# orottier/web-audio-api-rs

Hardware: AMD Instinct MI355X
Metric: render quanta/sec (48kHz, 128-frame) (higher is better)
Workload: dtype f64

## Files before the change

### web-audio-api-rs_amd/csrc/waa_biquad_stream.hip

```cpp
#include <hip/hip_runtime.h>

#include <cstdlib>

#include "waa_internal.hpp"
#include "waa_stream_common.hpp"

namespace waa {

namespace {
struct M2 {
  double a, b, c, d;
};
__device__ __forceinline__ M2 mm(const M2& x, const M2& y) {
  M2 r;
  r.a = __builtin_fma(x.a, y.a, x.b * y.c);
  r.b = __builtin_fma(x.a, y.b, x.b * y.d);
  r.c = __builtin_fma(x.c, y.a, x.d * y.c);
  r.d = __builtin_fma(x.c, y.b, x.d * y.d);
  return r;
}

}

__device__ unsigned long long g_stream_trace[8192 * 4];

template <int DBG, int VARY, int NBUF = 2, bool DUP = false>
__global__ __launch_bounds__(64, 2) void biquad_stream_kernel_t(const BiquadStreamDesc d) {
  extern __shared__ __attribute__((aligned(16))) float lds[];
  const uint32_t wid = blockIdx.x;
  const uint32_t inst = wid / (uint32_t)d.nch;
  const int ch = (int)(wid % (uint32_t)d.nch);
  const int lane = threadIdx.x;
  if (inst >= d.n_inst) return;

  __builtin_amdgcn_s_setreg(1 | (6 << 6) | (1 << 11), 0);
  unsigned long long trace_t0 = 0;
  if constexpr (DBG == 7) trace_t0 = wall_clock64();

  const double* cp = d.coefs + (uint64_t)inst * d.coef_stride;
  double b0 = cp[0], b1 = cp[1], b2 = cp[2], a1 = cp[3], a2 = cp[4];
  M2 A1;
  {
    M2 m = {-a1, -a2, 1., 0.};
#pragma unroll
    for (int s = 0; s < 5; s++) m = mm(m, m);
    A1 = m;
  }
  const M2 A2 = mm(A1, A1), A4 = mm(A2, A2), A8 = mm(A4, A4), A16 = mm(A8, A8);
  M2 Aj = {1., 0., 0., 1.};
  if constexpr (VARY == 0) {
    const int j = lane & 15;
    if (j & 1) Aj = mm(Aj, A1);
    if (j & 2) Aj = mm(Aj, A2);
    if (j & 4) Aj = mm(Aj, A4);
    if (j & 8) Aj = mm(Aj, A8);
  }
  const int row = lane >> 4;

  double* st = d.state + (uint64_t)inst * STATE_STRIDE + ch * 4;
  double cx1 = st[0], cx2 = st[1], cy1 = st[2], cy2 = st[3];

  float g[2] = {1.f, 1.f};
  bool g_mute[2] = {false, false}, g_pass[2] = {true, true};
#pragma unroll
  for (int k = 0; k < 2; k++)
    if (k < d.n_gain) {
      g[k] = d.gain[k].base[inst];
      g_mute[k] = fabsf(g[k]) <= 1e-6f;
      g_pass[k] = fabsf(1.f - g[k]) <= 1e-6f;
    }

  const bool is_src = d.in.kind == IN_SOURCE;
  SrcInst si{};
  SrcSchedule sc{};
  const float* sig_base = nullptr;
  if (is_src) {
    si = d.in.src[inst];
    sc = si.sc;
  } else {
    sig_base = d.in.sig.base + (uint64_t)inst * d.in.sig.inst_stride + (uint64_t)ch * d.in.sig.ch_stride;
  }
  float* out_base = d.out.base + (uint64_t)inst * d.out.inst_stride + (uint64_t)ch * d.out.ch_stride;

  auto lds_sync = []() __attribute__((always_inline)) { __builtin_amdgcn_wave_barrier(); };

  auto fetch_fast = [&](uint32_t tile, float (&dst)[TILE_K]) __attribute__((always_inline)) {
    const float* p = is_src ? si.base + (uint64_t)ch * si.ch_stride +
                                  (tile < si.fast_prefix ? si.linear_start + (int64_t)tile * TILE
                                                         : load_global(&sc.qrec[(uint64_t)tile * QUANTA_PER_TILE].start))
                            : sig_base + (uint64_t)tile * TILE;
#pragma unroll
    for (int j = 0; j < NV4; j++) {
      const f4v t = DBG == 5 ? load_global_f4(p + j * 256 + lane * 4)
                             : __builtin_nontemporal_load((const WAA_GLOBAL_AS f4v*)(p + j * 256 + lane * 4));
      dst[j * 4 + 0] = t.x;
      dst[j * 4 + 1] = t.y;
      dst[j * 4 + 2] = t.z;
      dst[j * 4 + 3] = t.w;
    }
  };
  auto tile_is_fast = [&](uint32_t tile) __attribute__((always_inline)) -> bool {
    return !is_src || tile < si.fast_prefix || (si.aligned && load_global(sc.tile_fast + tile));
  };

  auto stage = [&](const float (&cur)[TILE_K]) __attribute__((always_inline)) {
#pragma unroll
    for (int j = 0; j < NV4; j++) {
      const int r = j * 8 + (lane >> 3), c = (lane & 7) * 4;
      *reinterpret_cast<float4*>(lds + r * LDS_ROW + c) =
          make_float4(cur[j * 4 + 0], cur[j * 4 + 1], cur[j * 4 + 2], cur[j * 4 + 3]);
    }
  };
  float* lds_out = lds + 64 * LDS_ROW;
  auto flush = [&](uint32_t tile) __attribute__((always_inline)) {
    lds_sync();
    float* op = out_base + (uint64_t)tile * TILE;
#pragma unroll
    for (int j = 0; j < NV4; j++) {
      const int r = j * 8 + (lane >> 3), c = (lane & 7) * 4;
      float4 t = *reinterpret_cast<const float4*>(lds_out + r * LDS_ROW + c);
#pragma unroll
      for (int k = 0; k < 2; k++)
        if (k < d.n_gain) {
          if (g_mute[k]) {
            t = make_float4(0.f, 0.f, 0.f, 0.f);
          } else if (!g_pass[k]) {
            t.x *= g[k];
            t.y *= g[k];
            t.z *= g[k];
            t.w *= g[k];
          }
        }
      if constexpr (DBG == 2) {
        asm volatile("" ::"v"(t.x), "v"(t.y), "v"(t.z), "v"(t.w));
      } else if constexpr (DBG == 5) {
        *reinterpret_cast<float4*>(op + j * 256 + lane * 4) = t;
      } else {
        __builtin_nontemporal_store(f4v{t.x, t.y, t.z, t.w}, (WAA_GLOBAL_AS f4v*)(op + j * 256 + lane * 4));
        if constexpr (DUP)
          __builtin_nontemporal_store(f4v{t.x, t.y, t.z, t.w}, (WAA_GLOBAL_AS f4v*)(op + d.out.ch_stride + j * 256 + lane * 4));
      }
    }
    lds_sync();
  };
  auto process_arate = [&](uint32_t tile) __attribute__((always_inline)) {
    lds_sync();
    const float* xrow = lds + lane * LDS_ROW;
    float* yrow = lds_out + lane * LDS_ROW;
    const double* ct = cp + (uint64_t)tile * (TILE_K * 5 * 64) + lane;
    auto load_chunk = [&](double (&c)[20], int chunk) __attribute__((always_inline)) {
      if (DBG >= 3 && tile != d.tile0) return;
#pragma unroll
      for (int j = 0; j < 20; j++) c[j] = load_global(ct + (chunk * 20 + j) * 64);
    };
    const float xl1 = xrow[TILE_K - 1], xl2 = xrow[TILE_K - 2];
    const float xm1 = __shfl_up(xl1, 1, 64), xm2 = __shfl_up(xl2, 1, 64);
    const double xs1 = lane == 0 ? cx1 : (double)xm1, xs2 = lane == 0 ? cx2 : (double)xm2;
    double x1 = xs1, x2 = xs2, z1 = 0., z2 = 0.;
    M2 P = {1., 0., 0., 1.};
    double ca[20], cb[20], cc[NBUF == 3 ? 20 : 1];
    if constexpr (VARY == 3) {
      const double* hp = d.hp + (uint64_t)(DBG == 4 ? d.tile0 : tile) * (HP_WORDS * 64) + lane;
      load_chunk(ca, 0);
      load_chunk(cb, 1);
      double za = load_global(hp + 64 * 64) * xs1, zb = load_global(hp + 65 * 64) * xs1;
      double zc = load_global(hp + 66 * 64) * xs2, zd = load_global(hp + 67 * 64) * xs2;
#pragma unroll 2
      for (int chunk = 0; chunk < TILE_K / 4; chunk++) {
        const float4 xv = *reinterpret_cast<const float4*>(xrow + chunk * 4);
        const double* hc = hp + chunk * 8 * 64;
        const double h0 = load_global(hc), h1 = load_global(hc + 64), h2 = load_global(hc + 128), h3 = load_global(hc + 192),
                     h4 = load_global(hc + 256), h5 = load_global(hc + 320), h6 = load_global(hc + 384), h7 = load_global(hc + 448);
        za = __builtin_fma(h0, (double)xv.x, za);
        zb = __builtin_fma(h1, (double)xv.x, zb);
        zc = __builtin_fma(h2, (double)xv.y, zc);
        zd = __builtin_fma(h3, (double)xv.y, zd);
        za = __builtin_fma(h4, (double)xv.z, za);
        zb = __builtin_fma(h5, (double)xv.z, zb);
        zc = __builtin_fma(h6, (double)xv.w, zc);
        zd = __builtin_fma(h7, (double)xv.w, zd);
      }
      z1 = za + zc;
      z2 = zb + zd;
      P.a = load_global(hp + 68 * 64);
      P.b = load_global(hp + 69 * 64);
// ... 82 lines not shown
            p2 = p1;
            p1 = xd2;
            double y = (wi - c[j * 5 + 3] * y1) - c[j * 5 + 4] * y2;
            if (flush_bad && !__builtin_isnormal(y)) y = 0.;
            y2 = y1;
            y1 = y;
            yo[j] = (float)y;
            badacc = __builtin_fmaf(yo[j], 0.f, badacc);
          }
          *reinterpret_cast<float4*>(yrow + chunk * 4) = make_float4(yo[0], yo[1], yo[2], yo[3]);
        };
        if constexpr (NBUF == 3) {
#pragma unroll 1
          for (int chunk = 0; chunk < 6; chunk += 3) {
            load_chunk(cc, chunk + 2);
            step_b(ca, chunk);
            load_chunk(ca, chunk + 3);
            step_b(cb, chunk + 1);
            load_chunk(cb, chunk + 4);
            step_b(cc, chunk + 2);
          }
          step_b(ca, 6);
          step_b(cb, 7);
        } else {
#pragma unroll 1
          for (int chunk = 0; chunk < TILE_K / 4; chunk += 2) {
            step_b(ca, chunk);
            if (chunk + 2 < TILE_K / 4) load_chunk(ca, chunk + 2);
            step_b(cb, chunk + 1);
            if (chunk + 3 < TILE_K / 4) load_chunk(cb, chunk + 3);
          }
        }
      };
      sweep(false);
      if (__any(badacc != badacc)) {
        y1 = __builtin_isfinite(s1) ? s1 : 0.;
        y2 = __builtin_isfinite(s2) ? s2 : 0.;
        load_chunk(ca, 0);
        load_chunk(cb, 1);
        sweep(true);
      }
      cx1 = (double)__int_as_float(__builtin_amdgcn_readlane(__float_as_int(xl1), 63));
      cx2 = (double)__int_as_float(__builtin_amdgcn_readlane(__float_as_int(xl2), 63));
      cy1 = read_lane(y1, 63);
      cy2 = read_lane(y2, 63);
    }
    lds_sync();
  };
  auto process = [&](uint32_t tile) __attribute__((always_inline)) {
    lds_sync();
    float x[TILE_K];
#pragma unroll
    for (int j = 0; j < NV4; j++) {
      const float4 t = *reinterpret_cast<const float4*>(lds + lane * LDS_ROW + j * 4);
      x[j * 4 + 0] = t.x;
      x[j * 4 + 1] = t.y;
      x[j * 4 + 2] = t.z;
      x[j * 4 + 3] = t.w;
    }
    if constexpr (DBG == 1) {
      lds_sync();
#pragma unroll
      for (int j = 0; j < NV4; j++)
        *reinterpret_cast<float4*>(lds_out + lane * LDS_ROW + j * 4) =
            make_float4(x[j * 4 + 0], x[j * 4 + 1], x[j * 4 + 2], x[j * 4 + 3]);
      lds_sync();
      return;
    }
    M2 Al = A1;
    if constexpr (VARY == 1) {
      uint32_t q = tile * QUANTA_PER_TILE + (lane >> 2);
      if (q >= d.n_quanta) q = d.n_quanta - 1;
      const double* cq = cp + (uint64_t)q * 5;
      b0 = cq[0];
      b1 = cq[1];
      b2 = cq[2];
      a1 = cq[3];
      a2 = cq[4];
      M2 m = {-a1, -a2, 1., 0.};
#pragma unroll
      for (int s = 0; s < 5; s++) m = mm(m, m);
      Al = m;
    }
    const float xm1 = __shfl_up(x[TILE_K - 1], 1, 64), xm2 = __shfl_up(x[TILE_K - 2], 1, 64);
    double x1 = lane == 0 ? cx1 : (double)xm1;
    double x2 = lane == 0 ? cx2 : (double)xm2;
    double w[TILE_K];
    double z1 = 0., z2 = 0.;
#pragma unroll
    for (int i = 0; i < TILE_K; i++) {
      const double xd = (double)x[i];
      w[i] = (b0 * xd + b1 * x1) + b2 * x2;
      x2 = x1;
      x1 = xd;
      const double t = __builtin_fma(-a2, z2, w[i]);
      const double y = __builtin_fma(-a1, z1, t);
      z2 = z1;
      z1 = y;
    }
    double s1, s2;
    if constexpr (VARY == 0) {
      double r1 = z1, r2 = z2;
      {
        double q1 = row_shr<1>(r1), q2 = row_shr<1>(r2);
        r1 = __builtin_fma(A1.a, q1, __builtin_fma(A1.b, q2, r1));
        r2 = __builtin_fma(A1.c, q1, __builtin_fma(A1.d, q2, r2));
        q1 = row_shr<2>(r1);
        q2 = row_shr<2>(r2);
        r1 = __builtin_fma(A2.a, q1, __builtin_fma(A2.b, q2, r1));
        r2 = __builtin_fma(A2.c, q1, __builtin_fma(A2.d, q2, r2));
        q1 = row_shr<4>(r1);
        q2 = row_shr<4>(r2);
        r1 = __builtin_fma(A4.a, q1, __builtin_fma(A4.b, q2, r1));
        r2 = __builtin_fma(A4.c, q1, __builtin_fma(A4.d, q2, r2));
        q1 = row_shr<8>(r1);
        q2 = row_shr<8>(r2);
        r1 = __builtin_fma(A8.a, q1, __builtin_fma(A8.b, q2, r1));
        r2 = __builtin_fma(A8.c, q1, __builtin_fma(A8.d, q2, r2));
      }
      const double e01 = read_lane(r1, 15), e02 = read_lane(r2, 15);
      const double e11 = read_lane(r1, 31), e12 = read_lane(r2, 31);
      const double e21 = read_lane(r1, 47), e22 = read_lane(r2, 47);
      const double t01 = cy1, t02 = cy2;
      const double t11 = __builtin_fma(A16.a, t01, __builtin_fma(A16.b, t02, e01));
      const double t12 = __builtin_fma(A16.c, t01, __builtin_fma(A16.d, t02, e02));
      const double t21 = __builtin_fma(A16.a, t11, __builtin_fma(A16.b, t12, e11));
      const double t22 = __builtin_fma(A16.c, t11, __builtin_fma(A16.d, t12, e12));
      const double t31 = __builtin_fma(A16.a, t21, __builtin_fma(A16.b, t22, e21));
      const double t32 = __builtin_fma(A16.c, t21, __builtin_fma(A16.d, t22, e22));
      const double T1 = row == 0 ? t01 : row == 1 ? t11 : row == 2 ? t21 : t31;
      const double T2 = row == 0 ? t02 : row == 1 ? t12 : row == 2 ? t22 : t32;
      const double ex1 = row_shr<1>(r1), ex2 = row_shr<1>(r2);
      s1 = __builtin_fma(Aj.a, T1, __builtin_fma(Aj.b, T2, ex1));
      s2 = __builtin_fma(Aj.c, T1, __builtin_fma(Aj.d, T2, ex2));
    } else {
      M2 P = Al;
      double r1 = z1, r2 = z2;
      auto step = [&](auto shr) __attribute__((always_inline)) {
        M2 Q;
        Q.a = shr(P.a, 1.);
        Q.b = shr(P.b, 0.);
        Q.c = shr(P.c, 0.);
        Q.d = shr(P.d, 1.);
        const double q1 = shr(r1, 0.), q2 = shr(r2, 0.);
        r1 = __builtin_fma(P.a, q1, __builtin_fma(P.b, q2, r1));
        r2 = __builtin_fma(P.c, q1, __builtin_fma(P.d, q2, r2));
        P = mm(P, Q);
      };
      step([](double v, double idv) __attribute__((always_inline)) { return row_shr_keep<1>(v, idv); });
      step([](double v, double idv) __attribute__((always_inline)) { return row_shr_keep<2>(v, idv); });
      step([](double v, double idv) __attribute__((always_inline)) { return row_shr_keep<4>(v, idv); });
      step([](double v, double idv) __attribute__((always_inline)) { return row_shr_keep<8>(v, idv); });
      double t1[4], t2[4];
      t1[0] = cy1;
      t2[0] = cy2;
#pragma unroll
      for (int k = 0; k < 3; k++) {
        const int e = 16 * k + 15;
        const double pa = read_lane(P.a, e), pb = read_lane(P.b, e), pc = read_lane(P.c, e), pd = read_lane(P.d, e);
        const double e1 = read_lane(r1, e), e2 = read_lane(r2, e);
        t1[k + 1] = __builtin_fma(pa, t1[k], __builtin_fma(pb, t2[k], e1));
        t2[k + 1] = __builtin_fma(pc, t1[k], __builtin_fma(pd, t2[k], e2));
      }
      const double T1 = row == 0 ? t1[0] : row == 1 ? t1[1] : row == 2 ? t1[2] : t1[3];
      const double T2 = row == 0 ? t2[0] : row == 1 ? t2[1] : row == 2 ? t2[2] : t2[3];
      const double xa = row_shr_keep<1>(P.a, 1.), xb = row_shr_keep<1>(P.b, 0.), xc = row_shr_keep<1>(P.c, 0.),
                   xd = row_shr_keep<1>(P.d, 1.);
      const double x1r = row_shr_keep<1>(r1, 0.), x2r = row_shr_keep<1>(r2, 0.);
      s1 = __builtin_fma(xa, T1, __builtin_fma(xb, T2, x1r));
      s2 = __builtin_fma(xc, T1, __builtin_fma(xd, T2, x2r));
    }
    double y1 = s1, y2 = s2;
    float badacc = 0.f;
    float yo[TILE_K];
#pragma unroll
    for (int i = 0; i < TILE_K; i++) {
      const double y = (w[i] - a1 * y1) - a2 * y2;
      y2 = y1;
      y1 = y;
      yo[i] = (float)y;
      badacc = __builtin_fmaf(yo[i], 0.f, badacc);
    }
    if (__any(badacc != badacc)) {
      y1 = s1;
      y2 = s2;
      if (!__builtin_isfinite(y1)) y1 = 0.;
      if (!__builtin_isfinite(y2)) y2 = 0.;
#pragma unroll
      for (int i = 0; i < TILE_K; i++) {
        double y = (w[i] - a1 * y1) - a2 * y2;
        if (!__builtin_isnormal(y)) y = 0.;
        y2 = y1;
        y1 = y;
        yo[i] = (float)y;
      }
    }
    cx1 = (double)__int_as_float(__builtin_amdgcn_readlane(__float_as_int(x[TILE_K - 1]), 63));
    cx2 = (double)__int_as_float(__builtin_amdgcn_readlane(__float_as_int(x[TILE_K - 2]), 63));
    cy1 = read_lane(y1, 63);
    cy2 = read_lane(y2, 63);
    lds_sync();
#pragma unroll
    for (int j = 0; j < NV4; j++)
      *reinterpret_cast<float4*>(lds_out + lane * LDS_ROW + j * 4) =
          make_float4(yo[j * 4 + 0], yo[j * 4 + 1], yo[j * 4 + 2], yo[j * 4 + 3]);
    lds_sync();
  };

  bool pending = false;
  uint32_t pending_tile = 0;
  uint32_t tile = d.tile0;
  while (tile < d.tile1) {
    if (!tile_is_fast(tile)) {
      float tmp[TILE_K];
      load_channel_generic(d.in, si, sc, ch, tile, lane, d.n_quanta, tmp);
      float cur[TILE_K];
#pragma unroll
      for (int i = 0; i < TILE_K; i++) cur[i] = tmp[i];
      stage(cur);
      if (pending) flush(pending_tile);
      if constexpr (VARY >= 2) process_arate(tile); else process(tile);
      pending = true;
      pending_tile = tile;
      tile++;
      continue;
    }
    uint32_t end = tile + 1;
    if (is_src && end < si.fast_prefix) end = si.fast_prefix < d.tile1 ? si.fast_prefix : d.tile1;
    while (end < d.tile1 && tile_is_fast(end)) end++;
    if constexpr (VARY == 0 && NBUF == 4) {
      float na[TILE_K], nb[TILE_K];
      fetch_fast(tile, na);
      fetch_fast(tile + 1 < end ? tile + 1 : tile, nb);
      for (; tile + 1 < end; tile += 2) {
        stage(na);
        fetch_fast(tile + 2 < end ? tile + 2 : tile, na);
        if (pending) flush(pending_tile);
        process(tile);
        pending = true;
        pending_tile = tile;
        stage(nb);
        fetch_fast(tile + 3 < end ? tile + 3 : tile + 1, nb);
        flush(pending_tile);
        process(tile + 1);
        pending_tile = tile + 1;
      }
      if (tile < end) {
        stage(na);
        if (pending) flush(pending_tile);
        process(tile);
        pending = true;
        pending_tile = tile;
        tile++;
      }
      continue;
    }
    float nx[TILE_K];
    fetch_fast(tile, nx);
    for (; tile < end; tile++) {
      stage(nx);
      fetch_fast(tile + 1 < end ? tile + 1 : tile, nx);
      if (pending) flush(pending_tile);
      if constexpr (VARY >= 2) process_arate(tile); else process(tile);
      pending = true;
      pending_tile = tile;
    }
  }
  if (pending) flush(pending_tile);
  if (lane == 0) {
    st[0] = cx1;
    st[1] = cx2;
    st[2] = cy1;
    st[3] = cy2;
  }
  if constexpr (DBG == 7) {
    if (lane == 0 && wid < 8192) {
      g_stream_trace[wid * 4 + 0] = trace_t0;
      g_stream_trace[wid * 4 + 1] = wall_clock64();
      g_stream_trace[wid * 4 + 2] = __builtin_amdgcn_s_getreg(4 | (0 << 6) | (31 << 11));
      g_stream_trace[wid * 4 + 3] = __builtin_amdgcn_s_getreg(20 | (0 << 6) | (31 << 11));
    }
  }
}

__global__ __launch_bounds__(64, 4) void biquad_stream_digest_kernel(const BiquadStreamDesc d) {
  extern __shared__ __attribute__((aligned(16))) float lds[];
  double* htab = reinterpret_cast<double*>(lds + 64 * LDS_ROW);
  const uint32_t wid = blockIdx.x;
  const uint32_t inst = wid / (uint32_t)d.nch;
  const int ch = (int)(wid % (uint32_t)d.nch);
  const int lane = threadIdx.x;
  if (inst >= d.n_inst) return;
  __builtin_amdgcn_s_setreg(1 | (6 << 6) | (1 << 11), 0);

  auto uni = [](double v) __attribute__((always_inline)) {
    return __hiloint2double(__builtin_amdgcn_readfirstlane(__double2hiint(v)), __builtin_amdgcn_readfirstlane(__double2loint(v)));
  };
  auto uni_m = [&](const M2& m) __attribute__((always_inline)) { return M2{uni(m.a), uni(m.b), uni(m.c), uni(m.d)}; };
  const double* cp = d.coefs + (uint64_t)inst * d.coef_stride;
  const double b0 = uni(cp[0]), b1 = uni(cp[1]), b2 = uni(cp[2]), a1 = uni(cp[3]), a2 = uni(cp[4]);
  M2 A1;
  {
    M2 m = {-a1, -a2, 1., 0.};
#pragma unroll
    for (int s = 0; s < 5; s++) m = mm(m, m);
    A1 = uni_m(m);
  }
  const M2 A2 = uni_m(mm(A1, A1)), A4 = uni_m(mm(A2, A2)), A8 = uni_m(mm(A4, A4)), A16 = uni_m(mm(A8, A8));
  M2 Aj = {1., 0., 0., 1.};
  {
    const int j = lane & 15;
    if (j & 1) Aj = mm(Aj, A1);
    if (j & 2) Aj = mm(Aj, A2);
    if (j & 4) Aj = mm(Aj, A4);
    if (j & 8) Aj = mm(Aj, A8);
  }
  const int row = lane >> 4;
  {
    double g1 = 1., g2 = 0.;
    double p1 = 0., p2 = 0.;
    double q1 = 0., q2 = 0.;
    double h1 = 0., h2 = 0.;
    for (int n = 0; n < TILE_K; n++) {
      if (lane == TILE_K - 1 - n) {
        h1 = __builtin_fma(b0, g1, __builtin_fma(b1, p1, b2 * q1));
        h2 = __builtin_fma(b0, g2, __builtin_fma(b1, p2, b2 * q2));
      }
      if (n == TILE_K - 1) {
        if (lane == 32) {
          h1 = __builtin_fma(b1, g1, b2 * p1);
          h2 = __builtin_fma(b1, g2, b2 * p2);
        }
        if (lane == 33) {
          h1 = b2 * g1;
          h2 = b2 * g2;
        }
      }
      const double n1 = __builtin_fma(-a1, g1, -(a2 * g2)), n2 = g1;
      q1 = p1;
      q2 = p2;
      p1 = g1;
      p2 = g2;
      g1 = n1;
      g2 = n2;
    }
    if (lane < 34) {
      htab[lane * 2] = h1;
      htab[lane * 2 + 1] = h2;
    }
  }
  double* st = d.state + (uint64_t)inst * STATE_STRIDE + ch * 4;
  double cx1 = st[0], cx2 = st[1], cy1 = st[2], cy2 = st[3];
  float g[2] = {1.f, 1.f};
  bool g_mute[2] = {false, false}, g_pass[2] = {true, true};
#pragma unroll
  for (int k = 0; k < 2; k++)
    if (k < d.n_gain) {
      g[k] = d.gain[k].base[inst];
      g_mute[k] = fabsf(g[k]) <= 1e-6f;
      g_pass[k] = fabsf(1.f - g[k]) <= 1e-6f;
    }
  const bool is_src = d.in.kind == IN_SOURCE;
  SrcInst si{};
  SrcSchedule sc{};
  const float* sig_base = nullptr;
// ... 159 lines not shown
      }
      if (__any(badacc != badacc)) {
        y1 = sy1;
        y2 = sy2;
        p1 = sp1;
        p2 = sp2;
#pragma unroll
        for (int j = 0; j < 4; j++) {
          const double xd = (double)xf[j];
          const double wi = (b0 * xd + b1 * p1) + b2 * p2;
          p2 = p1;
          p1 = xd;
          double y = (wi - a1 * y1) - a2 * y2;
          if (!__builtin_isnormal(y)) y = 0.;
          y2 = y1;
          y1 = y;
          yo[j] = (float)y;
        }
      }
      *reinterpret_cast<float4*>(xrow + c * 4) = make_float4(yo[0], yo[1], yo[2], yo[3]);
    }
    cx1 = (double)__int_as_float(__builtin_amdgcn_readlane(__float_as_int(xl1), 63));
    cx2 = (double)__int_as_float(__builtin_amdgcn_readlane(__float_as_int(xl2), 63));
    cy1 = read_lane(y1, 63);
    cy2 = read_lane(y2, 63);
  };
  bool have = false;
  uint32_t done = 0;
  uint32_t tile = d.tile0;
  while (tile < d.tile1) {
    if (!tile_is_fast(tile)) {
      float tmp[TILE_K];
      load_channel_generic(d.in, si, sc, ch, tile, lane, d.n_quanta, tmp);
      float cur[TILE_K];
#pragma unroll
      for (int i = 0; i < TILE_K; i++) cur[i] = tmp[i];
      swap_in(cur, have, done);
      process();
      have = true;
      done = tile;
      tile++;
      continue;
    }
    uint32_t end = tile + 1;
    if (is_src && end < si.fast_prefix) end = si.fast_prefix < d.tile1 ? si.fast_prefix : d.tile1;
    while (end < d.tile1 && tile_is_fast(end)) end++;
    float nx[TILE_K];
    fetch_fast(tile, nx);
    for (; tile < end; tile++) {
      swap_in(nx, have, done);
      fetch_fast(tile + 1 < end ? tile + 1 : tile, nx);
      process();
      have = true;
      done = tile;
    }
  }
  if (have) flush_last(done);
  if (lane == 0) {
    st[0] = cx1;
    st[1] = cx2;
    st[2] = cy1;
    st[3] = cy2;
  }
}

void launch_biquad_stream(const BiquadStreamDesc& d, void* stream) {
  const dim3 grid(d.n_inst * (uint32_t)d.nch), block(64);
  const size_t lds = 2 * 64 * LDS_ROW * sizeof(float);
  const char* dbg = measure_switch("WAA_STREAM_DEBUG");
  if (d.dup_out && d.vary == 0) {
    hipLaunchKernelGGL((biquad_stream_kernel_t<0, 0, 4, true>), grid, block, lds, (hipStream_t)stream, d);
    return;
  }
  if (d.vary == 3 && dbg && dbg[0] == '3')
    hipLaunchKernelGGL((biquad_stream_kernel_t<3, 3>), grid, block, lds, (hipStream_t)stream, d);
  else if (d.vary == 3 && dbg && dbg[0] == '4')
    hipLaunchKernelGGL((biquad_stream_kernel_t<4, 3>), grid, block, lds, (hipStream_t)stream, d);
  else if (d.vary == 3 && measure_switch("WAA_ARATE_BUFS3"))
    hipLaunchKernelGGL((biquad_stream_kernel_t<0, 3, 3>), grid, block, lds, (hipStream_t)stream, d);
  else if (d.vary == 3)
    hipLaunchKernelGGL((biquad_stream_kernel_t<0, 3>), grid, block, lds, (hipStream_t)stream, d);
  else if (d.vary == 2)
    hipLaunchKernelGGL((biquad_stream_kernel_t<0, 2>), grid, block, lds, (hipStream_t)stream, d);
  else if (d.vary)
    hipLaunchKernelGGL((biquad_stream_kernel_t<0, 1>), grid, block, lds, (hipStream_t)stream, d);
  else if (dbg && dbg[0] == '1')
    hipLaunchKernelGGL((biquad_stream_kernel_t<1, 0>), grid, block, lds, (hipStream_t)stream, d);
  else if (dbg && dbg[0] == '2')
    hipLaunchKernelGGL((biquad_stream_kernel_t<2, 0>), grid, block, lds, (hipStream_t)stream, d);
  else if (dbg && dbg[0] == '5')
    hipLaunchKernelGGL((biquad_stream_kernel_t<5, 0>), grid, block, lds, (hipStream_t)stream, d);
  else if (dbg && dbg[0] == '7')
    hipLaunchKernelGGL((biquad_stream_kernel_t<7, 0>), grid, block, lds, (hipStream_t)stream, d);
  else if (measure_switch("WAA_STREAM_PREFETCH1"))
    hipLaunchKernelGGL((biquad_stream_kernel_t<0, 0, 2>), grid, block, lds, (hipStream_t)stream, d);
  else if (measure_switch("WAA_BIQUAD_DIGEST"))
    hipLaunchKernelGGL(biquad_stream_digest_kernel, grid, block, 64 * LDS_ROW * sizeof(float) + 34 * 2 * sizeof(double),
                       (hipStream_t)stream, d);
  else
    hipLaunchKernelGGL((biquad_stream_kernel_t<0, 0, 4>), grid, block, lds, (hipStream_t)stream, d);
}

}

extern "C" int waa_debug_stream_trace(unsigned long long* dst, unsigned n_words) {
  return (int)hipMemcpyFromSymbol(dst, HIP_SYMBOL(waa::g_stream_trace), (size_t)n_words * 8);
}
```

### web-audio-api-rs_amd/csrc/waa_internal.hpp

```cpp
#pragma once
#include <cstdint>
#include <cstdlib>

#include "waa_conv_noise.hpp"

namespace waa {

inline const char* measure_switch(const char* name) {
#ifdef WAA_MEASURE
  return getenv(name);
#else
  (void)name;
  return nullptr;
#endif
}

void raise_lds_limit(const void* kernel);

constexpr int RQ = 128;
constexpr int TILE_K = 32;
constexpr int TILE = 64 * TILE_K;
constexpr int QUANTA_PER_TILE = TILE / RQ;
constexpr int MAX_OPS = 12;
constexpr int MAX_INPUTS = 4;
// ... 37 lines not shown
  uint64_t frames;
  uint32_t sched;
  uint32_t aligned;
  SrcSchedule sc;
  int64_t linear_start;
  uint32_t fast_prefix;
  uint32_t linear_all;
};

enum : int32_t { IN_SILENT = 0, IN_SIGNAL = 1, IN_SOURCE = 2, IN_CONSTANT = 3, IN_DELAYED = 4 };
struct InputRef {
  int32_t kind;
  int32_t nch;
  SignalRef sig;
  const SrcInst* src;
  const SrcSchedule* sched;
  ParamRef offset;
  const int64_t* active;
  double sample_rate;
  int32_t num_quanta;
  int32_t feedback;
  uint64_t valid;
  ParamRef gain;
  int32_t has_gain;
  uint32_t fast_tiles;
  float delay_lo, delay_hi;
};

enum : int32_t {
  OP_GAIN = 1,
  OP_BIQUAD = 2,
  OP_WAVESHAPER = 3,
  OP_STEREO_PAN = 4,
  OP_PANNER = 5,
  OP_MIX = 6,
  OP_IIR = 7,
  OP_PARAM_ADD = 8
};
struct OpDesc {
  int32_t kind;
  int32_t nch_in;
  int32_t nch_out;
  int32_t i1;
  int32_t i2;
  int32_t i0;
  ParamRef p0;
  ParamRef p1;
  ParamRef p2;
  ParamRef p3;
  ParamRef p4;
  const void* ptr0;
  void* ptr1;
  const void* ptr2;
  uint64_t u0;
};

struct ChainDesc {
  int32_t n_inputs;
  int32_t in_nch;
  int32_t in_interp;
  int32_t n_ops;
  InputRef in[MAX_INPUTS];
  OpDesc ops[MAX_OPS];
  SignalRef out;
  uint32_t n_inst;
  uint32_t n_tiles;
  uint32_t n_quanta;
  uint32_t xcd_remap;
  uint32_t tile0, tile1;
  int32_t lds_curve_op;
  int32_t tile_major;
  uint32_t persist_block;
  uint32_t pad;
};

struct BiquadStreamDesc {
  InputRef in;
  const double* coefs;
  uint64_t coef_stride;
  int32_t vary;
  int32_t pad0;
  double* state;
  const double* hp;
  ParamRef gain[2];
  int32_t n_gain;
  int32_t nch;
  SignalRef out;
  uint32_t n_inst;
  uint32_t n_tiles;
  uint32_t n_quanta;
  uint32_t dup_out;
  uint32_t tile0, tile1;
};
void launch_biquad_stream(const BiquadStreamDesc& d, void* stream);
constexpr int BIQUAD_SCAN_PW = 88;
struct BiquadScanCtl {
  uint32_t* counter;
  uint32_t counter_base[8];
  double* payload;
  const double* pw;
  uint32_t* error;
};
void launch_biquad_scan_powers(const double* coefs, uint64_t coef_stride, double* pw, uint32_t n_inst, void* stream);
void launch_biquad_scan(const BiquadStreamDesc& d, const BiquadScanCtl& ctl, uint32_t* issued, void* stream);

constexpr int BIQUAD_HT_WORDS = 2 * TILE + 8;
struct BiquadLanesDesc {
  InputRef in;
  const double* coefs;
  double* ht;
  double* z;
  double* sin;
  double* state;
  ParamRef gain[2];
  int32_t n_gain, nch;
  SignalRef out;
  uint32_t n_inst, n_tiles, n_quanta, tile0, tile1;
  uint32_t fast_tiles;
  uint32_t lt0, lt1;
  uint32_t debug, pad;
};
void launch_biquad_tile_digest(const BiquadLanesDesc& d, void* stream);
void launch_biquad_lanes(const BiquadLanesDesc& d, void* stream);

struct IirStreamDesc {
  InputRef in;
  const double* coef;
  const double* pow;
  double* state;
  int32_t ns;
  int32_t nch;
  SignalRef out;
  uint32_t n_inst;
  uint32_t n_tiles;
  uint32_t n_quanta;
  uint32_t exact;
  uint32_t tile0, tile1;
};
int iir_padded_states(int n_states);
void launch_iir_stream(const IirStreamDesc& d, void* stream);

struct CompRow {
  float thr, lo, hi, half_knee;
  float knee_partial, ratio, makeup, pad;
  float a_tau, a_one, r_tau, r_one;
};
struct CompDesc {
  SignalRef in;
  uint64_t in_valid;
  SignalRef out;
  float* xl;
  const CompRow* rows;
  uint32_t row_inst_stride, row_q_stride;
  uint32_t n_inst, n_quanta;
  uint64_t frames;
  uint32_t delay_frames;
  int32_t nch;
};
void launch_compressor_level(const CompDesc& d, void* stream);
void launch_compressor_detector(const CompDesc& d, void* stream);
void launch_compressor_apply(const CompDesc& d, void* stream);

enum : int32_t { RT_CHANNEL = 0, RT_DOWN2 = 1, RT_DOWN4 = 2, RT_DOWN6 = 3 };
struct RouteTerm {
  const float* base;
  uint64_t inst_stride, ch_stride;
  int32_t mode;
  int32_t ch;
};
struct RouteDesc {
  SignalRef out;
  const RouteTerm* terms;
  const uint32_t* row_off;
  uint32_t n_inst, rows;
  uint64_t frames;
};
void launch_route(const RouteDesc& d, void* stream);
// ... 514 lines not shown
```

### web-audio-api-rs_amd/csrc/waa_plan.cpp

```cpp
#include <array>
#include <set>

#include <memory>

#include "waa_host.hpp"
#include "waa_plan_parts.hpp"

namespace waa {
namespace host {

int prepare_source_input(waa_batch* b, uint32_t id, InputRef* in);
int validate_plan(waa_batch* b);

int device_timeline_param(waa_batch* b, const ParamStore& p, ParamRef* ref) {
  if (p.dev_ready) {
    *ref = p.dev_ref;
    return 0;
  }
  std::vector<TlHeader> hdr(b->n_inst);
  std::vector<TlEvent> events;
  std::vector<float> curves;
  for (uint32_t i = 0; i < b->n_inst; i++) {
    TlHeader& h = hdr[i];
    std::memset(&h, 0, sizeof h);
// ... 675 lines not shown
      in.kind = IN_SIGNAL;
      in.nch = cur_nch;
      in.sig = seg_out;
      inputs.assign(1, in);
      in_nch = cur_nch;
      i = j;
      if (i == ops.size() && seg_out.base == out.base) return 0;
      continue;
    }
    if (o.kind == OP_BIQUAD && o.i0 == 2 && !dup && b->steps[(size_t)o.i1].coef.rows == 1 && !measure_switch("WAA_ARATE_STREAM") &&
        (inputs[0].kind == IN_SIGNAL || inputs[0].kind == IN_SOURCE) &&
        (uint64_t)b->n_inst * seg_out.inst_stride < (1ull << 32)) {
      Step& cstep = b->steps[(size_t)o.i1];
      Step& dstep = b->steps[(size_t)o.i1 + 1];
      cstep.coef.lane_major = 0;
      const size_t n_streams = (size_t)b->n_inst * cur_nch;
      double *ht = nullptr, *z = nullptr, *sin = nullptr;
      int e;
      if ((e = dev_alloc(b, &ht, (size_t)b->n_tiles * BIQUAD_HT_WORDS)) || (e = dev_alloc(b, &z, (size_t)b->n_tiles * n_streams * 2)) ||
          (e = dev_alloc(b, &sin, (size_t)b->n_tiles * n_streams * 2)))
        return e;
      BiquadLanesDesc L;
      std::memset(&L, 0, sizeof L);
      L.in = inputs[0];
      L.coefs = cstep.coef.coefs;
      L.ht = ht;
      L.z = z;
      L.sin = sin;
      L.state = reinterpret_cast<double*>(o.ptr1);
      L.n_gain = (int)(j - i - 1);
      for (size_t k = i + 1; k < j; k++) L.gain[k - i - 1] = ops[k].p0;
      L.nch = cur_nch;
      L.out = seg_out;
      L.n_inst = b->n_inst;
      L.n_tiles = b->n_tiles;
      L.n_quanta = b->n_quanta;
      L.tile0 = 0;
      L.tile1 = b->n_tiles;
      L.fast_tiles = inputs[0].kind == IN_SOURCE ? inputs[0].fast_tiles
                                                 : (inputs[0].valid ? (uint32_t)std::min<uint64_t>(inputs[0].valid / TILE, b->n_tiles) : b->n_tiles);
      dstep.kind = 18;
      dstep.lanes = L;
      dstep.profile_slot = slot_for(b, "biquad_tile_digest_kernel");
      Step ls;
      ls.kind = 19;
      ls.lanes = L;
      ls.profile_slot = slot_for(b, "biquad_lanes_kernel");
      b->steps.push_back(ls);
      plan_note(b, "biquad_lanes(a-rate, shared table: one lane per stream, tiles in parallel) in=%s:%dch gains=%d out=%s",
                input_kind_name(inputs[0].kind), cur_nch, L.n_gain, seg_out.base == out.base ? "final" : "temp");
      InputRef in{};
      in.kind = IN_SIGNAL;
      in.nch = cur_nch;
      in.sig = seg_out;
      inputs.assign(1, in);
      in_nch = cur_nch;
      i = j;
      if (i == ops.size() && seg_out.base == out.base) return 0;
      continue;
    }
    Step st;
    st.kind = 1;
    BiquadStreamDesc& q = st.bq;
    std::memset(&q, 0, sizeof q);
    q.in = inputs[0];
    q.coefs = reinterpret_cast<const double*>(o.ptr0);
    q.coef_stride = o.u0;
    q.vary = o.i0;
    if (o.i0 == 2) {
      Step& cstep = b->steps[(size_t)o.i1];
      cstep.coef.lane_major = 1;
      if (cstep.coef.rows == 1 && !measure_switch("WAA_NO_ARATE_DIGEST")) {
        Step& hstep = b->steps[(size_t)o.i1 + 1];
        double* dhp = nullptr;
        int e = dev_alloc(b, &dhp, (size_t)b->n_tiles * HP_WORDS * 64);
        if (e) return e;
        hstep.hp.coefs = cstep.coef.coefs;
        hstep.hp.hp = dhp;
        hstep.hp.n_tiles = b->n_tiles;
        q.hp = dhp;
        q.vary = 3;
      }
    }
    q.state = reinterpret_cast<double*>(o.ptr1);
    q.n_gain = (int)(j - i - 1);
    for (size_t k = i + 1; k < j; k++) q.gain[k - i - 1] = ops[k].p0;
    q.nch = cur_nch;
    q.out = seg_out;
    q.dup_out = dup ? 1u : 0u;
    q.n_inst = b->n_inst;
    q.n_tiles = b->n_tiles;
    q.tile0 = 0;
    q.tile1 = b->n_tiles;
    q.n_quanta = b->n_quanta;
    st.profile_slot = slot_for(b, "biquad_stream_kernel");
    if (q.vary == 0 && !b->dry && measure_switch("WAA_BIQUAD_SCAN")) {
      const size_t n_streams = (size_t)b->n_inst * cur_nch;
      if (!b->scan_counter) {
        int e = dev_alloc(b, &b->scan_counter, 8 * 16 + 16);
        if (e) return e;
        b->state_bufs.push_back({b->scan_counter, (8 * 16 + 16) * sizeof(uint32_t)});
      }
      double *payload = nullptr, *pw = nullptr;
      int e;
      if ((e = dev_alloc(b, &payload, n_streams * b->n_tiles * 8)) || (e = dev_alloc(b, &pw, (size_t)b->n_inst * BIQUAD_SCAN_PW)))
        return e;
      b->ones_bufs.push_back({payload, n_streams * b->n_tiles * 8 * sizeof(double)});
      launch_biquad_scan_powers(q.coefs, q.coef_stride, pw, b->n_inst, b->stream);
      HIP_TRY(hipGetLastError());
      st.scan.counter = b->scan_counter;
      st.scan.error = b->scan_counter + 8 * 16;
      st.scan.payload = payload;
      st.scan.pw = pw;
      st.profile_slot = slot_for(b, "biquad_scan_kernel");
    }
    b->steps.push_back(st);
    if (dup) {
      plan_note(b, "biquad_stream in=%s:1ch gains=%d out=final (both channels: the speakers up-mix 1 -> 2 behind it)",
                input_kind_name(inputs[0].kind), q.n_gain);
      return 0;
    }
    plan_note(b, "biquad_stream%s in=%s:%dch gains=%d out=%s",
              q.vary == 3 ? "(a-rate, shared table)" : q.vary == 2 ? "(a-rate, per-instance table)" : q.vary ? "(k-rate)" : "",
              input_kind_name(inputs[0].kind),
              cur_nch, q.n_gain, seg_out.base == out.base ? "final" : "temp");
    InputRef in{};
    in.kind = IN_SIGNAL;
    in.nch = cur_nch;
    in.sig = seg_out;
    inputs.assign(1, in);
    in_nch = cur_nch;
    i = j;
    if (i == ops.size() && seg_out.base == out.base) return 0;
  }
  return push_chain_step(b, inputs, in_nch, in_interp, pending, out);
}

bool is_delay(const waa_batch* b, uint32_t id) { return b->nodes[id].desc.kind == WAA_NODE_DELAY; }
void vertex_targets(const waa_batch* b, uint32_t v, const std::vector<uint8_t>& cut, std::vector<uint32_t>& out) {
  const uint32_t id = v & ~VTX_READER;
  if (!(v & VTX_READER) && is_delay(b, id)) {
    if (!cut[id]) out.push_back(id | VTX_READER);
    return;
  }
  for (auto& e : b->edges) {
    if (e.from != id) continue;
    out.push_back(is_delay(b, e.to) && (e.to_input & 0x80000000u) ? (e.to | VTX_READER) : e.to);
  }
}

int materialise_automation(waa_batch* b) {
  const double sample_rate = (double)b->sr, dt = 1. / sample_rate;
  for (Node& n : b->nodes)
    for (size_t pk = 0; pk < n.params.size(); pk++) {
      ParamStore& p = n.params[pk];
      if (p.timelines.empty()) continue;
      bool shared = p.timelines_shared && p.timelines[0];
      for (uint32_t i = 1; i < b->n_inst && shared; i++) shared = p.cst[i] == p.cst[0] && p.timelines[i];
      {
        const uint32_t kind = n.desc.kind;
        const bool consumable = kind == WAA_NODE_GAIN || kind == WAA_NODE_BIQUAD || kind == WAA_NODE_DELAY ||
                                kind == WAA_NODE_STEREO_PANNER || kind == WAA_NODE_CONSTANT_SOURCE ||
                                kind == WAA_NODE_OSCILLATOR ||
                                (kind == WAA_NODE_PANNER && pk >= 6 && n.desc.i[0] != WAA_PANNING_HRTF);
        const bool want = measure_switch("WAA_DEVICE_AUTOMATION") ? true : !shared;
        bool arrivals = false;
// ... 1312 lines not shown
```

### web-audio-api-rs_amd/csrc/waa_plan_ops.cpp

```cpp
#include <array>
#include <set>

#include "waa_host.hpp"
#include "waa_plan_parts.hpp"

namespace waa {
namespace host {

int emit_node_ops(waa_batch* b, uint32_t id, int cur_nch, bool head, std::vector<OpDesc>& ops, int* out_nch) {
  Node& n = b->nodes[id];
  const uint32_t kind = n.desc.kind;
  if (kind == WAA_NODE_BUFFER_SOURCE || kind == WAA_NODE_CONSTANT_SOURCE) {
    *out_nch = n.out_nch;
    return 0;
  }
  if (!head && cur_nch != n.in_nch) {
    OpDesc m{};
    m.kind = OP_MIX;
    m.nch_in = cur_nch;
    m.nch_out = n.in_nch;
    m.i0 = n.interp;
    ops.push_back(m);
  }
  const int nch = n.in_nch;
  *out_nch = n.out_nch;
  switch (kind) {
    case WAA_NODE_GAIN: {
      OpDesc o{};
      o.kind = OP_GAIN;
      o.nch_in = o.nch_out = nch;
      int e = node_param(b, id, 0, &o.p0);
      if (e) return e;
      ops.push_back(o);
      break;
    }
    case WAA_NODE_BIQUAD: {
      OpDesc o{};
      o.kind = OP_BIQUAD;
      o.nch_in = o.nch_out = nch;
      bool varies = false, a_rate = false;
      for (size_t k = 0; k < n.params.size(); k++) {
        if (param_mode(n, k) == 2) a_rate = true;
        if (param_mode(n, k) == 1) varies = true;
      }
      if (a_rate) {
        Step cs;
        cs.kind = 5;
        BiquadCoefDesc& cdsc = cs.coef;
        std::memset(&cdsc, 0, sizeof cdsc);
        int e;
        if ((e = node_param(b, id, WAA_PARAM_BIQUAD_FREQUENCY, &cdsc.frequency)) ||
            (e = node_param(b, id, WAA_PARAM_BIQUAD_DETUNE, &cdsc.detune)) ||
            (e = node_param(b, id, WAA_PARAM_BIQUAD_Q, &cdsc.q)) ||
            (e = node_param(b, id, WAA_PARAM_BIQUAD_GAIN, &cdsc.gain)))
          return e;
        cdsc.n_frames = (uint64_t)b->n_quanta * RQ;
        cdsc.frames_padded = b->lp;
        bool shared = true;
        for (size_t k = 0; k < 4; k++) {
          const bool modulated = k < n.pin_edges.size() && !n.pin_edges[k].empty();
          const ParamStore& ps = n.params[k];
          if (modulated || ps.dev_tl) shared = false;
          for (uint32_t i = 1; i < b->n_inst && shared; i++) shared = ps.cst[i] == ps.cst[0];
          for (auto& blk : ps.blocks) shared &= blk.inst == WAA_ALL_INSTANCES;
        }
        cdsc.rows = shared ? 1u : b->n_inst;
        cdsc.type = n.desc.i[0];
        cdsc.sample_rate = b->sr;
        double* dco = nullptr;
        if ((e = dev_alloc(b, &dco, (size_t)cdsc.rows * cdsc.frames_padded * 5))) return e;
        cdsc.coefs = dco;
        cs.profile_slot = slot_for(b, "biquad_coef_kernel");
        b->steps.push_back(cs);
        double* dst = nullptr;
        if ((e = dev_alloc(b, &dst, (size_t)b->n_inst * STATE_STRIDE))) return e;
        b->state_bufs.push_back({dst, (size_t)b->n_inst * STATE_STRIDE * sizeof(double)});
        o.i0 = 2;
        o.i1 = (int32_t)b->steps.size() - 1;
        {
          Step hs;
          hs.kind = 12;
          std::memset(&hs.hp, 0, sizeof hs.hp);
          hs.profile_slot = slot_for(b, "biquad_hp_kernel");
          b->steps.push_back(hs);
        }
        o.ptr0 = dco;
        o.ptr1 = dst;
        o.u0 = shared ? 0 : cdsc.frames_padded * 5;
        ops.push_back(o);
        break;
      }
      const uint64_t per = varies ? (uint64_t)b->n_quanta * 5 : 5;
      std::vector<double> co((size_t)b->n_inst * per);
      std::vector<float> pf, pd, pq, pg;
      for (uint32_t i = 0; i < b->n_inst; i++) {
        auto f = param_per_quantum(b, n.params[WAA_PARAM_BIQUAD_FREQUENCY], i, nullptr);
        auto d = param_per_quantum(b, n.params[WAA_PARAM_BIQUAD_DETUNE], i, nullptr);
        auto q = param_per_quantum(b, n.params[WAA_PARAM_BIQUAD_Q], i, nullptr);
        auto g = param_per_quantum(b, n.params[WAA_PARAM_BIQUAD_GAIN], i, nullptr);
        if (i > 0 && f == pf && d == pd && q == pq && g == pg) {
          std::copy(co.begin() + (size_t)(i - 1) * per, co.begin() + (size_t)i * per, co.begin() + (size_t)i * per);
          continue;
        }
        pf = f;
        pd = d;
        pq = q;
        pg = g;
        const uint32_t cnt = varies ? b->n_quanta : 1;
        for (uint32_t k = 0; k < cnt; k++) {
          auto at = [&](const std::vector<float>& v) { return v[v.size() == 1 ? 0 : k]; };
          Coefs c = biquad_coefs(n.desc.i[0], (double)b->sr, (double)computed_freq(at(f), at(d)), (double)at(g), (double)at(q));
          double* dst = &co[(size_t)i * per + (size_t)k * 5];
          dst[0] = c.b0;
          dst[1] = c.b1;
          dst[2] = c.b2;
          dst[3] = c.a1;
          dst[4] = c.a2;
        }
      }
      double* dco = nullptr;
      int e = dev_upload(b, &dco, co);
      if (e) return e;
      double* dst = nullptr;
      e = dev_alloc(b, &dst, (size_t)b->n_inst * STATE_STRIDE);
      if (e) return e;
      b->state_bufs.push_back({dst, (size_t)b->n_inst * STATE_STRIDE * sizeof(double)});
      o.i0 = varies ? 1 : 0;
      o.ptr0 = dco;
      o.ptr1 = dst;
      o.u0 = per;
      ops.push_back(o);
      break;
    }
    case WAA_NODE_IIR_FILTER: {
      OpDesc o{};
      o.kind = OP_IIR;
      o.nch_in = o.nch_out = nch;
      const int len = (int)n.iir_b.size();
      const int ns = iir_padded_states(len - 1);
      if (ns < 0) return fail(WAA_ERR_DEVICE, "internal: IIR order");
      std::vector<double> co(2 * (size_t)(ns + 1), 0.);
      for (int k = 0; k < len; k++) {
        co[k] = n.iir_b[k];
        co[ns + 1 + k] = n.iir_a[k];
      }
      std::vector<DD> m((size_t)ns * ns), t((size_t)ns * ns);
      for (int i = 0; i < ns; i++) {
        m[(size_t)i * ns] = DD{-co[ns + 1 + i + 1], 0.};
        if (i + 1 < ns) m[(size_t)i * ns + i + 1] = dd_add(m[(size_t)i * ns + i + 1], DD{1., 0.});
      }
      double growth = 0.;
      auto note = [&](const std::vector<DD>& a) {
        for (const DD& v : a) growth = std::isfinite(v.hi) ? std::max(growth, std::fabs(v.hi)) : INFINITY;
      };
      auto mul = [&](const std::vector<DD>& x, const std::vector<DD>& y, std::vector<DD>& out) {
        for (int r = 0; r < ns; r++)
          for (int c = 0; c < ns; c++) {
            DD acc{0., 0.};
            for (int k = 0; k < ns; k++) acc = dd_add(acc, dd_mul(x[(size_t)r * ns + k], y[(size_t)k * ns + c]));
            out[(size_t)r * ns + c] = acc;
          }
      };
      for (int k = 0; k < 5; k++) {
        mul(m, m, t);
        m.swap(t);
        note(m);
      }
      const std::vector<DD> A = m;
      std::vector<double> pw(6 * (size_t)ns * ns);
      for (int lvl = 0; lvl < 6; lvl++) {
        for (size_t k = 0; k < (size_t)ns * ns; k++) pw[lvl * (size_t)ns * ns + k] = m[k].hi + m[k].lo;
        mul(m, m, t);
        m.swap(t);
        note(m);
      }
      m = A;
      for (int j = 2; j <= 64 && std::isfinite(growth); j++) {
        mul(m, A, t);
        m.swap(t);
        note(m);
      }
      const char* genv = measure_switch("WAA_IIR_GROWTH");
      const double growth_limit = genv ? atof(genv) : 1e4;
      const bool exact = !(growth <= growth_limit) || getenv("WAA_IIR_EXACT") != nullptr;
      if (exact)
        for (auto& v : pw) v = 0.;
      double *dco = nullptr, *dpw = nullptr, *dst = nullptr;
      int e;
      if ((e = dev_upload(b, &dco, co)) || (e = dev_upload(b, &dpw, pw))) return e;
      const size_t n_state = (size_t)b->n_inst * nch * ns;
      if ((e = dev_alloc(b, &dst, n_state))) return e;
      b->state_bufs.push_back({dst, n_state * sizeof(double)});
      o.i0 = exact ? -ns : ns;
      o.ptr0 = dco;
      o.ptr1 = dst;
      o.ptr2 = dpw;
      ops.push_back(o);
      break;
    }
    case WAA_NODE_WAVESHAPER: {
      if (n.has_curve) {
        OpDesc o{};
        o.kind = OP_WAVESHAPER;
        o.nch_in = o.nch_out = nch;
        if (!n.d_curve) {
          int e = dev_upload(b, &n.d_curve, n.curve);
          if (e) return e;
        }
        o.ptr0 = n.d_curve;
        o.i0 = (int)n.curve.size();
        ops.push_back(o);
      }
      break;
// ... 187 lines not shown
```

Before: 2.931 billion.

## Precompute k-rate biquad scan matrices into a shared per-tile table

When every instance shares one k-rate coefficient row, the host uploads that row only once. A new kernel precomputes the per-tile scan matrix powers (A^32 and the prefix-doubling products) into a table at plan time. The stream kernel gets a VARY==4 variant that loads these from the table instead of doing repeated 2x2 matrix squaring and multiplication per tile. The cost is extra table memory traffic per tile and an added prologue/prefetch path for the coefficients.

Result: no change. 2.916 billion (-0.5%).

```diff
diff --git a/web-audio-api-rs_amd/csrc/waa_biquad_stream.hip b/web-audio-api-rs_amd/csrc/waa_biquad_stream.hip
--- a/web-audio-api-rs_amd/csrc/waa_biquad_stream.hip
+++ b/web-audio-api-rs_amd/csrc/waa_biquad_stream.hip
@@ -20,6 +20,7 @@
   return r;
 }
 
+__device__ __forceinline__ double load_uniform(const double* p) { return *(const __attribute__((address_space(4))) double*)p; }
 }
 
 __device__ unsigned long long g_stream_trace[8192 * 4];
@@ -101,6 +102,18 @@
   };
   auto tile_is_fast = [&](uint32_t tile) __attribute__((always_inline)) -> bool {
     return !is_src || tile < si.fast_prefix || (si.aligned && load_global(sc.tile_fast + tile));
+  };
+
+  double kc[5], kt[KTAB_LANE_WORDS];
+  auto fetch_k = [&](uint32_t tile) __attribute__((always_inline)) {
+    uint32_t q = tile * QUANTA_PER_TILE + (lane >> 2);
+    if (q >= d.n_quanta) q = d.n_quanta - 1;
+    const double* cq = cp + (uint64_t)q * 5;
+#pragma unroll
+    for (int j = 0; j < 5; j++) kc[j] = load_global(cq + j);
+    const double* tp = d.ktab + (uint64_t)tile * KTAB_WORDS + lane;
+#pragma unroll
+    for (int j = 0; j < KTAB_LANE_WORDS; j++) kt[j] = load_global(tp + j * 64);
   };
 
   auto stage = [&](const float (&cur)[TILE_K]) __attribute__((always_inline)) {
@@ -349,6 +362,17 @@
       for (int s = 0; s < 5; s++) m = mm(m, m);
       Al = m;
     }
+    double rc[VARY == 4 ? 12 : 1];
+    if constexpr (VARY == 4) {
+      b0 = kc[0];
+      b1 = kc[1];
+      b2 = kc[2];
+      a1 = kc[3];
+      a2 = kc[4];
+      const double* rp = d.ktab + (uint64_t)__builtin_amdgcn_readfirstlane(tile) * KTAB_WORDS + KTAB_LANE_WORDS * 64;
+#pragma unroll
+      for (int j = 0; j < 12; j++) rc[j] = load_uniform(rp + j);
+    }
     const float xm1 = __shfl_up(x[TILE_K - 1], 1, 64), xm2 = __shfl_up(x[TILE_K - 2], 1, 64);
     double x1 = lane == 0 ? cx1 : (double)xm1;
     double x2 = lane == 0 ? cx2 : (double)xm2;
@@ -400,6 +424,32 @@
       const double ex1 = row_shr<1>(r1), ex2 = row_shr<1>(r2);
       s1 = __builtin_fma(Aj.a, T1, __builtin_fma(Aj.b, T2, ex1));
       s2 = __builtin_fma(Aj.c, T1, __builtin_fma(Aj.d, T2, ex2));
+    } else if constexpr (VARY == 4) {
+      double r1 = z1, r2 = z2;
+      auto step = [&](auto shr, const double* P) __attribute__((always_inline)) {
+        const double q1 = shr(r1, 0.), q2 = shr(r2, 0.);
+        r1 = __builtin_fma(P[0], q1, __builtin_fma(P[1], q2, r1));
+        r2 = __builtin_fma(P[2], q1, __builtin_fma(P[3], q2, r2));
+      };
+      step([](double v, double idv) __attribute__((always_inline)) { return row_shr_keep<1>(v, idv); }, kt);
+      step([](double v, double idv) __attribute__((always_inline)) { return row_shr_keep<2>(v, idv); }, kt + 4);
+      step([](double v, double idv) __attribute__((always_inline)) { return row_shr_keep<4>(v, idv); }, kt + 8);
+      step([](double v, double idv) __attribute__((always_inline)) { return row_shr_keep<8>(v, idv); }, kt + 12);
+      double t1[4], t2[4];
+      t1[0] = cy1;
+      t2[0] = cy2;
+#pragma unroll
+      for (int k = 0; k < 3; k++) {
+        const int e = 16 * k + 15;
+        const double e1 = read_lane(r1, e), e2 = read_lane(r2, e);
+        t1[k + 1] = __builtin_fma(rc[k * 4], t1[k], __builtin_fma(rc[k * 4 + 1], t2[k], e1));
+        t2[k + 1] = __builtin_fma(rc[k * 4 + 2], t1[k], __builtin_fma(rc[k * 4 + 3], t2[k], e2));
+      }
+      const double T1 = row == 0 ? t1[0] : row == 1 ? t1[1] : row == 2 ? t1[2] : t1[3];
+      const double T2 = row == 0 ? t2[0] : row == 1 ? t2[1] : row == 2 ? t2[2] : t2[3];
+      const double x1r = row_shr_keep<1>(r1, 0.), x2r = row_shr_keep<1>(r2, 0.);
+      s1 = __builtin_fma(kt[16], T1, __builtin_fma(kt[17], T2, x1r));
+      s2 = __builtin_fma(kt[18], T1, __builtin_fma(kt[19], T2, x2r));
     } else {
       M2 P = Al;
       double r1 = z1, r2 = z2;
@@ -485,8 +535,9 @@
 #pragma unroll
       for (int i = 0; i < TILE_K; i++) cur[i] = tmp[i];
       stage(cur);
+      if constexpr (VARY == 4) fetch_k(tile);
       if (pending) flush(pending_tile);
-      if constexpr (VARY >= 2) process_arate(tile); else process(tile);
+      if constexpr (VARY == 2 || VARY == 3) process_arate(tile); else process(tile);
       pending = true;
       pending_tile = tile;
       tile++;
@@ -524,11 +575,23 @@
     }
     float nx[TILE_K];
     fetch_fast(tile, nx);
+    if constexpr (VARY == 4) {
+      if (!pending) {
+        stage(nx);
+        fetch_k(tile);
+        fetch_fast(tile + 1 < end ? tile + 1 : tile, nx);
+        process(tile);
+        pending = true;
+        pending_tile = tile;
+        tile++;
+      }
+    }
     for (; tile < end; tile++) {
       stage(nx);
+      if constexpr (VARY == 4) fetch_k(tile);
       fetch_fast(tile + 1 < end ? tile + 1 : tile, nx);
       if (pending) flush(pending_tile);
-      if constexpr (VARY >= 2) process_arate(tile); else process(tile);
+      if constexpr (VARY == 2 || VARY == 3) process_arate(tile); else process(tile);
       pending = true;
       pending_tile = tile;
     }
@@ -548,6 +611,61 @@
       g_stream_trace[wid * 4 + 3] = __builtin_amdgcn_s_getreg(20 | (0 << 6) | (31 << 11));
     }
   }
+}
+
+__global__ __launch_bounds__(64) void biquad_ktab_kernel(const double* coefs, double* ktab, uint32_t n_quanta, uint32_t n_tiles) {
+  const uint32_t tile = blockIdx.x;
+  const int lane = threadIdx.x;
+  if (tile >= n_tiles) return;
+  __builtin_amdgcn_s_setreg(1 | (6 << 6) | (1 << 11), 0);
+  uint32_t q = tile * QUANTA_PER_TILE + (lane >> 2);
+  if (q >= n_quanta) q = n_quanta - 1;
+  const double* cq = coefs + (uint64_t)q * 5;
+  const double a1 = cq[3], a2 = cq[4];
+  M2 m = {-a1, -a2, 1., 0.};
+#pragma unroll
+  for (int s = 0; s < 5; s++) m = mm(m, m);
+  M2 P = m;
+  double* tp = ktab + (uint64_t)tile * KTAB_WORDS;
+  auto put = [&](int e, const M2& v) __attribute__((always_inline)) {
+    tp[(e + 0) * 64 + lane] = v.a;
+    tp[(e + 1) * 64 + lane] = v.b;
+    tp[(e + 2) * 64 + lane] = v.c;
+    tp[(e + 3) * 64 + lane] = v.d;
+  };
+  auto step = [&](auto shr) __attribute__((always_inline)) {
+    M2 Q;
+    Q.a = shr(P.a, 1.);
+    Q.b = shr(P.b, 0.);
+    Q.c = shr(P.c, 0.);
+    Q.d = shr(P.d, 1.);
+    P = mm(P, Q);
+  };
+  put(0, P);
+  step([](double v, double idv) __attribute__((always_inline)) { return row_shr_keep<1>(v, idv); });
+  put(4, P);
+  step([](double v, double idv) __attribute__((always_inline)) { return row_shr_keep<2>(v, idv); });
+  put(8, P);
+  step([](double v, double idv) __attribute__((always_inline)) { return row_shr_keep<4>(v, idv); });
+  put(12, P);
+  step([](double v, double idv) __attribute__((always_inline)) { return row_shr_keep<8>(v, idv); });
+  M2 X;
+  X.a = row_shr_keep<1>(P.a, 1.);
+  X.b = row_shr_keep<1>(P.b, 0.);
+  X.c = row_shr_keep<1>(P.c, 0.);
+  X.d = row_shr_keep<1>(P.d, 1.);
+  put(16, X);
+  if ((lane & 15) == 15 && lane < 48) {
+    double* rp = tp + KTAB_LANE_WORDS * 64 + (lane >> 4) * 4;
+    rp[0] = P.a;
+    rp[1] = P.b;
+    rp[2] = P.c;
+    rp[3] = P.d;
+  }
+}
+
+void launch_biquad_ktab(const double* coefs, double* ktab, uint32_t n_quanta, uint32_t n_tiles, void* stream) {
+  hipLaunchKernelGGL(biquad_ktab_kernel, dim3(n_tiles), dim3(64), 0, (hipStream_t)stream, coefs, ktab, n_quanta, n_tiles);
 }
 
 __global__ __launch_bounds__(64, 4) void biquad_stream_digest_kernel(const BiquadStreamDesc d) {
@@ -873,6 +991,8 @@
     hipLaunchKernelGGL((biquad_stream_kernel_t<0, 3>), grid, block, lds, (hipStream_t)stream, d);
   else if (d.vary == 2)
     hipLaunchKernelGGL((biquad_stream_kernel_t<0, 2>), grid, block, lds, (hipStream_t)stream, d);
+  else if (d.vary && d.ktab && d.coef_stride == 0)
+    hipLaunchKernelGGL((biquad_stream_kernel_t<0, 4>), grid, block, lds, (hipStream_t)stream, d);
   else if (d.vary)
     hipLaunchKernelGGL((biquad_stream_kernel_t<0, 1>), grid, block, lds, (hipStream_t)stream, d);
   else if (dbg && dbg[0] == '1')
diff --git a/web-audio-api-rs_amd/csrc/waa_internal.hpp b/web-audio-api-rs_amd/csrc/waa_internal.hpp
--- a/web-audio-api-rs_amd/csrc/waa_internal.hpp
+++ b/web-audio-api-rs_amd/csrc/waa_internal.hpp
@@ -143,6 +143,7 @@
   int32_t pad0;
   double* state;
   const double* hp;
+  const double* ktab;
   ParamRef gain[2];
   int32_t n_gain;
   int32_t nch;
@@ -154,6 +155,9 @@
   uint32_t tile0, tile1;
 };
 void launch_biquad_stream(const BiquadStreamDesc& d, void* stream);
+constexpr int KTAB_LANE_WORDS = 20;
+constexpr int KTAB_WORDS = KTAB_LANE_WORDS * 64 + 16;
+void launch_biquad_ktab(const double* coefs, double* ktab, uint32_t n_quanta, uint32_t n_tiles, void* stream);
 constexpr int BIQUAD_SCAN_PW = 88;
 struct BiquadScanCtl {
   uint32_t* counter;
diff --git a/web-audio-api-rs_amd/csrc/waa_plan.cpp b/web-audio-api-rs_amd/csrc/waa_plan.cpp
--- a/web-audio-api-rs_amd/csrc/waa_plan.cpp
+++ b/web-audio-api-rs_amd/csrc/waa_plan.cpp
@@ -781,6 +781,20 @@
         q.vary = 3;
       }
     }
+    if (o.i0 == 1 && o.u0 == 0 && !measure_switch("WAA_KRATE_INLINE_SCAN")) {
+      double* kt = nullptr;
+      int e = dev_alloc(b, &kt, (size_t)b->n_tiles * KTAB_WORDS);
+      if (e) return e;
+      if (!b->dry) {
+        launch_biquad_ktab(q.coefs, kt, b->n_quanta, b->n_tiles, b->stream);
+        HIP_TRY(hipGetLastError());
+      }
+      q.ktab = kt;
+      plan_note(b, "k-rate scan table: one coefficient row for all instances, %u tiles x %d doubles, formed once per plan", b->n_tiles,
+                KTAB_WORDS);
+    } else if (o.i0 == 1) {
+      plan_note(b, "k-rate scan inline: %s", o.u0 ? "a coefficient row per instance" : "one coefficient row, the table switched off");
+    }
     q.state = reinterpret_cast<double*>(o.ptr1);
     q.n_gain = (int)(j - i - 1);
     for (size_t k = i + 1; k < j; k++) q.gain[k - i - 1] = ops[k].p0;
diff --git a/web-audio-api-rs_amd/csrc/waa_plan_ops.cpp b/web-audio-api-rs_amd/csrc/waa_plan_ops.cpp
--- a/web-audio-api-rs_amd/csrc/waa_plan_ops.cpp
+++ b/web-audio-api-rs_amd/csrc/waa_plan_ops.cpp
@@ -93,6 +93,7 @@
       const uint64_t per = varies ? (uint64_t)b->n_quanta * 5 : 5;
       std::vector<double> co((size_t)b->n_inst * per);
       std::vector<float> pf, pd, pq, pg;
+      bool one_row = varies;
       for (uint32_t i = 0; i < b->n_inst; i++) {
         auto f = param_per_quantum(b, n.params[WAA_PARAM_BIQUAD_FREQUENCY], i, nullptr);
         auto d = param_per_quantum(b, n.params[WAA_PARAM_BIQUAD_DETUNE], i, nullptr);
@@ -102,6 +103,7 @@
           std::copy(co.begin() + (size_t)(i - 1) * per, co.begin() + (size_t)i * per, co.begin() + (size_t)i * per);
           continue;
         }
+        if (i > 0) one_row = false;
         pf = f;
         pd = d;
         pq = q;
@@ -118,6 +120,7 @@
           dst[4] = c.a2;
         }
       }
+      if (one_row) co.resize((size_t)per);
       double* dco = nullptr;
       int e = dev_upload(b, &dco, co);
       if (e) return e;
@@ -128,7 +131,7 @@
       o.i0 = varies ? 1 : 0;
       o.ptr0 = dco;
       o.ptr1 = dst;
-      o.u0 = per;
+      o.u0 = one_row ? 0 : per;
       ops.push_back(o);
       break;
     }
```
